# XuyangBai/D3Feat.pytorch

Hardware: AMD Instinct MI355X
Metric: fragment-pairs/sec (fwd+bwd) on 3DMatch-shaped pairs (higher is better)
Workload: dtype f32

## Files before the change

### d3feat.pytorch_amd/_native.py

```python
import ctypes as C
import os
import subprocess

_PKG_DIR = os.path.dirname(os.path.abspath(__file__))
_REPO = os.path.dirname(_PKG_DIR)
LIB_PATH = os.path.join(_PKG_DIR, "libd3feat_hip.so")
CSRC = os.path.join(_PKG_DIR, "csrc")
SOURCES = ["radius_neighbors.hip", "grid_subsample.hip", "kpconv.hip", "kpconv_fused.hip", "kpconv_aggregate.hip", "kpconv_small.hip", "kpconv_deform.hip", "pool.hip", "detection.hip", "loss.hip",
           "reverse_table.hip", "kpconv_dx_gather.hip", "matching.hip", "elementwise.hip", "batchnorm.hip", "linear.hip", "gemm_epilogue.hip", "optimizer.hip", "misc.hip",
           "registration.hip"]

_vp, _i, _f, _sz = C.c_void_p, C.c_int, C.c_float, C.c_size_t


class Tunables(C.Structure):
    _fields_ = [("atb_task_us", C.c_int32), ("atb_form", C.c_int32), ("atb_first_form_wgs", C.c_int32),
                ("match_wgs", C.c_int32), ("agg_through_lds", C.c_int32), ("atb_pipe", C.c_int32), ("xw_rows", C.c_int32), ("xw_split", C.c_int32),
                ("rowgemm_wide", C.c_int32), ("rowgemm_rt", C.c_int32), ("reserved", C.c_int32 * 6)]


class AtbProblem(C.Structure):
    _fields_ = [("x", _vp), ("grad_out", _vp), ("grad_w", _vp), ("N", C.c_int32), ("Cin", C.c_int32),
                ("Cout", C.c_int32), ("ldw", C.c_int32), ("bias_part", _vp), ("bias_blocks", C.c_int32),
                ("bias_cols", C.c_int32), ("grad_bias", _vp), ("grad_bias2", _vp)]


SIGNATURES = {
    "d3f_version": (C.c_char_p, []),
    "d3f_device_arch_ok": (_i, []),
    "d3f_device_arch_name": (_i, [C.c_char_p, _i]),
    "d3f_debug_set_flags": (None, [_i]),
    "d3f_get_tunables": (None, [C.POINTER(Tunables)]),
    "d3f_set_tunables": (_i, [C.POINTER(Tunables)]),
    "d3f_linear_grad_weight_group_ws_bytes": (_sz, [C.POINTER(AtbProblem), _i]),
    "d3f_linear_grad_weight_group": (_i, [C.POINTER(AtbProblem), _i, _vp, _sz, _vp]),
    "d3f_debug_set_phase_clock": (None, [_vp]),
    "d3f_debug_kernel_timing_begin": (_i, [_i, _i]),
    "d3f_debug_kernel_timing_end": (_i, [_vp, _vp, _i]),
    "d3f_radius_grid_ws_bytes": (_sz, [_i]),
    "d3f_radius_grid_build": (_i, [_vp, _i, _vp, _i, _f, _vp, _sz, _vp, _vp]),
    "d3f_radius_query": (_i, [_vp, _vp, _i, _vp, _vp, _i, _vp, _i, _f, _i, _vp, _vp, _vp, _vp, _vp]),
# ... 31 lines not shown
    "d3f_kpconv_aggregate_modes": (_i, [_vp, _i, _vp, _i, _vp, _i, _vp, _i, _vp, _i, _f, _i, _vp, _vp, _vp]),
    "d3f_kpconv_grad_input_modes": (_i, [_vp, _i, _vp, _i, _vp, _i, _i, _vp, _i, _f, _i, _vp, _vp, _vp]),
    "d3f_kpconv_grad_input": (_i, [_vp, _i, _vp, _i, _vp, _i, _vp, _i, _vp, _i, _f, _vp, _vp, _i, _vp, _vp, _sz, _vp]),
    "d3f_kpconv_aggregate_transposed_supported": (_i, [_i, _i]),
    "d3f_kpconv_aggregate_transposed": (_i, [_vp, _i, _i, _i, _vp, _i, _f, _vp, _vp, _i, _vp, _vp]),
    "d3f_reverse_table_ws_bytes": (_sz, [_i, _i, _i]),
    "d3f_reverse_table_build": (_i, [_vp, _i, _i, _i, _vp, _vp, _vp, _sz, _vp]),
    "d3f_kpconv_grad_input_gather_supported": (_i, [_i, _i, _i]),
    "d3f_kpconv_grad_input_gather": (_i, [_vp, _i, _vp, _i, _vp, _vp, _vp, _i, _f, _vp, _vp, _i, _vp, _i, _i, _f, _vp, _vp, _vp,
                                          _vp, _vp]),
    "d3f_reverse_table_filter": (_i, [_vp, _i, _vp, _vp, _i, _vp, _i, _f, _vp, _vp, _vp]),
    "d3f_linear_grad_weight_supported": (_i, [_i, _i, _i]),
    "d3f_linear_fused_supported": (_i, [_i, _i, _i]),
    "d3f_linear_bias_act_forward": (_i, [_vp, _vp, _i, _i, _i, _vp, _vp, _vp, _f, _vp, _vp, _i, _vp]),
    "d3f_linear_pair_supported": (_i, [_i, _i, _i, _i]),
    "d3f_linear_pair_bias_act_forward": (_i, [_vp, _vp, _i, _vp, _vp, _i, _i, _i, _vp, _vp, _vp, _vp, _f, _vp, _vp, _i, _vp]),
    "d3f_linear_grad_input": (_i, [_vp, _vp, _i, _i, _i, _vp, _vp, _vp]),
    "d3f_linear_grad_weight_ws_bytes": (_sz, [_i, _i, _i]),
    "d3f_linear_grad_weight": (_i, [_vp, _vp, _i, _i, _i, _vp, _vp, _sz, _vp]),
    "d3f_linear_grad_weight_bias": (_i, [_vp, _vp, _i, _i, _i, _vp, _vp, _sz, _vp, _i, _i, _vp, _vp, _vp]),
    "d3f_permute_kpconv_weights": (_i, [_vp, _vp, _vp, _vp, _vp, _i, _vp]),
    "d3f_gemm_epilogue_supported": (_i, [_i, _i, _i, _i, _i]),
    "d3f_gemm_epilogue_ws_bytes": (_sz, [_i, _i, _i]),
    "d3f_gemm_epilogue": (_i, [_vp, _i, _vp, _i, _i, _i, _i, _i, _i, _vp, _vp, _vp, _i, _vp, _f, _vp, _i, _vp, _i, _vp, _sz,
                               _vp]),
    "d3f_bias_act_backward_blocks": (_i, [_i, _i]),
    "d3f_bias_act_backward_partial": (_i, [_vp, _vp, _f, _i, _i, _vp, _vp, _vp, _sz, _vp]),
    "d3f_bias_sum": (_i, [_vp, _i, _i, _vp, _vp, _vp]),
    "d3f_max_pool_forward": (_i, [_vp, _i, _i, _vp, _i, _i, _vp, _vp, _vp, _vp, _vp, _i, _i, _vp]),
    "d3f_max_pool_backward": (_i, [_vp, _vp, _i, _i, _i, _vp, _i, _vp]),
    "d3f_closest_pool_forward": (_i, [_vp, _i, _i, _vp, _i, _i, _vp, _i, _vp, _vp, _vp]),
    "d3f_closest_pool_backward": (_i, [_vp, _i, _vp, _i, _i, _i, _i, _vp, _i, _vp]),
    "d3f_bias_act_forward": (_i, [_vp, _vp, _vp, _vp, _f, _i, _i, _vp, _vp, _i, _vp, _vp, _i, _i, _vp]),
    "d3f_bias_act_backward_ws_bytes": (_sz, [_i, _i]),
    "d3f_bias_act_backward": (_i, [_vp, _vp, _f, _i, _i, _vp, _vp, _vp, _i, _vp, _vp, _sz, _vp]),
    "d3f_global_max": (_i, [_vp, _sz, _vp, _vp, _sz, _vp]),
    "d3f_global_max_rows": (_i, [_vp, _i, _i, _vp, _i, _vp, _vp, _sz, _vp]),
    "d3f_global_max_groups": (_i, [_vp, _i, _i, _vp, _i, _i, _vp, _vp, _sz, _vp]),
    "d3f_detection_scores_aux_floats": (_i, [_i]),
    "d3f_detection_scores_forward": (_i, [_vp, _i, _i, _vp, _i, _vp, _i, _vp, _vp, _vp, _vp, _i, _i, _vp]),
    "d3f_detection_scores_ws_bytes": (_sz, [_i, _i]),
    "d3f_detection_scores_backward": (_i, [_vp, _i, _i, _vp, _i, _vp, _vp, _vp, _vp, _vp, _sz, _vp]),
    "d3f_detection_scores_backward_groups": (_i, [_vp, _i, _i, _vp, _i, _vp, _vp, _vp, _vp, _vp, _i, _i, _vp, _sz, _vp]),
    "d3f_circle_det_loss_forward_pairs": (_i, [_vp, _vp, _i, _i, _i, _vp, _vp, _vp, _f, _f, _f, _f, _f, _f, _vp, _vp, _vp,
                                               _vp, _vp, _vp, _vp]),
    "d3f_circle_det_loss_backward_pairs": (_i, [_vp, _vp, _i, _i, _i, _vp, _vp, _vp, _f, _f, _f, _f, _f, _f, _vp, _vp,
# ... 98 lines not shown
        _lib = handle
    return _lib


TRACE = False


def check(rc, what):
    if TRACE:
        import sys
        import torch
        sys.stderr.write("[d3f] %s\n" % what)
        sys.stderr.flush()
        torch.cuda.synchronize()
    if rc != 0:
        raise RuntimeError("%s failed: %s" % (what, ERRORS.get(rc, "error %d" % rc)))


def set_tunables(**kw):
    L = lib()
    t = Tunables()
    L.d3f_get_tunables(C.byref(t))
    old = {name: getattr(t, name) for name, _ in Tunables._fields_ if name != "reserved"}
    for k, v in kw.items():
        if k not in old:
            raise RuntimeError("d3f_tunables has no field %r" % k)
        setattr(t, k, int(v))
    check(L.d3f_set_tunables(C.byref(t)), "d3f_set_tunables")
    return old


def status_message(word):
    return "; ".join(msg for bit, msg in STATUS_BITS.items() if word & bit)
```

### d3feat.pytorch_amd/csrc/gemm_epilogue.hip

```cpp
#include <math.h>

#include "kpconv_tile.hpp"

namespace d3f {

namespace {

constexpr int XW_RING_BYTES = 16 * 1024;
constexpr int XW_LDS_BYTES = 4 * XW_RING_BYTES;

struct XwArgs {
  const float* X;
  const float* W;
  float* Y;
  float* part;
  const float* row_div;
  const float* b1;
  const float* add;
  const float* b2;
  float* zinit;
  int R, Kd, N;
  int lda, ldb, ldy, ldadd;
  int kblock;
  int P, kpp;
// ... 224 lines not shown
  for (int q = 0; q < TI; ++q) {
    const int s = wave * TI + q, i = s >> 2, r = s & 3;
    const int row = m0 + 16 * i + 4 * lk + r;
    float v[TJ];
#pragma unroll
    for (int u = 0; u < TJ; ++u) {
      const int e = ((i * TJ + u) * 4 + r) * 64 + lane;
      v[u] = ((red[e] + red[NT * 256 + e]) + red[2 * NT * 256 + e]) + red[3 * NT * 256 + e];
    }
    if (row < g.R) {
      const int col = n0 + TJ * li;
      if (g.P == 1) {
        xw_epilogue_store<TJ>(v, g, row, col);
      } else {
        float* dst = g.part + ((size_t)p * g.R + row) * g.N + col;
        if constexpr (TJ == 4) *(float4*)dst = make_float4(v[0], v[TJ > 1 ? 1 : 0], v[TJ > 2 ? 2 : 0], v[TJ > 3 ? 3 : 0]);
        else if constexpr (TJ == 2) *(float2*)dst = make_float2(v[0], v[TJ > 1 ? 1 : 0]);
        else dst[0] = v[0];
      }
    }
  }
}

__global__ __launch_bounds__(256) void xw_reduce_epilogue_kernel(const XwArgs g) {
  const size_t e4 = (size_t)blockIdx.x * 256 + threadIdx.x;
  const size_t total4 = (size_t)g.R * g.N / 4;
  if (e4 >= total4) return;
  const float4* part4 = (const float4*)g.part;
  float4 s = part4[e4];
  for (int p = 1; p < g.P; ++p) {
    const float4 w = part4[(size_t)p * total4 + e4];
    s.x += w.x; s.y += w.y; s.z += w.z; s.w += w.w;
  }
  const uint32_t e = (uint32_t)e4 * 4u, row = e / (uint32_t)g.N, col = e - row * (uint32_t)g.N;
  float v[4] = {s.x, s.y, s.z, s.w};
  xw_epilogue_store<4>(v, g, (int)row, (int)col);
}

static inline int xw_tile_width(int n) { return n % 64 == 0 ? 4 : (n % 32 == 0 ? 2 : (n % 16 == 0 ? 1 : 0)); }

struct XwPlan {
  int ti, tj, nrb, nbj, P, kpp;
  unsigned grid;
  size_t slab_floats;
};

}

bool xw_supported(int R, int Kd, int N, int mode, int kblock) {
  if (R < 1 || Kd < 16 || Kd % 16 || N < 16 || !xw_tile_width(N) || mode < 0 || mode > 1) return false;
  if (kblock != 0 && (mode != 0 || kblock < 64 || kblock % 64 || Kd % kblock)) return false;
  if (((size_t)R + 64) * (size_t)Kd * 4 >= 0xfff00000ull || ((size_t)N + 64) * (size_t)Kd * 4 >= 0xfff00000ull) return false;
  if ((size_t)R * N >= 0x3fffffffull) return false;
  return true;
}

static XwPlan xw_plan(int R, int Kd, int N) {
  XwPlan a;
  const d3f_tunables& tn = tunables();
  a.tj = xw_tile_width(N);
  a.nbj = N / (16 * a.tj);
  a.ti = 4;
  if ((long long)cdiv(R, 64) * a.nbj < 512) a.ti = 2;
  if (tn.xw_rows == 2 || tn.xw_rows == 4) a.ti = tn.xw_rows;
  a.nrb = cdiv(R, 16 * a.ti);
  const long long ntiles = (long long)a.nrb * a.nbj;
  a.P = 1;
  if (ntiles <= 160 && Kd >= 1024 && Kd % 128 == 0) a.P = 8;
  if (tn.xw_split == 1) a.P = 1;
  if (tn.xw_split >= 8 && tn.xw_split % 8 == 0 && Kd % (16 * tn.xw_split) == 0) a.P = tn.xw_split;
  a.kpp = a.P == 1 ? Kd : Kd / a.P;
  a.grid = a.P == 1 ? (unsigned)(8 * ((ntiles + 7) / 8)) : (unsigned)(a.P * ntiles);
  a.slab_floats = a.P == 1 ? 0 : (size_t)a.P * R * N;
  return a;
}

size_t xw_ws_bytes(int R, int Kd, int N) {
  return 256 + align_up(sizeof(float) * xw_plan(R, Kd, N).slab_floats, 256);
}

int xw_gemm(const float* X, int lda, const float* W, int ldb, int mode, int kblock, int R, int Kd, int N,
            const float* row_div, const float* b1, const float* add, int ldadd, const float* b2, float slope, float* Y,
            int ldy, float* zinit, int zn, void* ws, size_t ws_bytes, hipStream_t stream) {
  if (!X || !W || !Y || !xw_supported(R, Kd, N, mode, kblock)) return D3F_EINVAL;
  if (lda < Kd || ldy < N || (add && ldadd < N) || (zinit && zn < 1)) return D3F_EINVAL;
  if (mode == 0 && kblock == 0 && ldb < Kd) return D3F_EINVAL;
  if (mode == 1 && ldb < N) return D3F_EINVAL;
  if ((((uintptr_t)X | (uintptr_t)W | (uintptr_t)Y | (uintptr_t)add | (uintptr_t)b1 | (uintptr_t)b2) & 15) != 0) return D3F_EINVAL;
  if ((lda | ldb | ldy | (add ? ldadd : 0)) & 3) return D3F_EINVAL;
  const XwPlan pl = xw_plan(R, Kd, N);
  if (pl.P > 1 && (!ws || ws_bytes < xw_ws_bytes(R, Kd, N))) return D3F_EWORKSPACE;
  XwArgs g;
  g.X = X; g.W = W; g.Y = Y;
  g.part = pl.P > 1 ? (float*)ws : nullptr;
  g.row_div = row_div; g.b1 = b1; g.add = add; g.b2 = b2;
  g.zinit = zinit; g.zn = zinit ? zn : 0;
  g.R = R; g.Kd = Kd; g.N = N;
  g.lda = lda; g.ldb = (mode == 0 && kblock > 0) ? kblock : ldb; g.ldy = ldy; g.ldadd = add ? ldadd : 0;
  g.kblock = kblock;
  g.P = pl.P; g.kpp = pl.kpp;
  g.nrb = pl.nrb; g.nbj = pl.nbj;
  g.slope = slope;
  const size_t bx = (size_t)R * lda * 4;
  const size_t bw = mode == 1 ? (size_t)Kd * ldb * 4 : (kblock > 0 ? (size_t)Kd * N * 4 : (size_t)N * ldb * 4);
  if (bx >= 0xfff00000ull || bw >= 0xfff00000ull) return D3F_EINVAL;
  g.bytesX = (unsigned)bx;
  g.bytesW = (unsigned)bw;
#define D3F_XW(I, J, M) \
  case (M) * 64 + (I) * 8 + (J): xw_gemm_kernel<I, J, M><<<pl.grid, 256, XW_LDS_BYTES, stream>>>(g); break
  switch (mode * 64 + pl.ti * 8 + pl.tj) {
    D3F_XW(2, 1, 0); D3F_XW(2, 2, 0); D3F_XW(2, 4, 0); D3F_XW(4, 1, 0); D3F_XW(4, 2, 0); D3F_XW(4, 4, 0);
    D3F_XW(2, 1, 1); D3F_XW(2, 2, 1); D3F_XW(2, 4, 1); D3F_XW(4, 1, 1); D3F_XW(4, 2, 1); D3F_XW(4, 4, 1);
    default: return D3F_EINVAL;
  }
#undef D3F_XW
  D3F_LAUNCH_CHECK();
  if (pl.P > 1) {
    xw_reduce_epilogue_kernel<<<cdiv((long long)R * N / 4, 256), 256, 0, stream>>>(g);
    D3F_LAUNCH_CHECK();
  }
  return D3F_OK;
}

}

extern "C" {

int d3f_gemm_epilogue_supported(int R, int K, int N, int mode, int kblock) {
  return d3f::xw_supported(R, K, N, mode, kblock) ? 1 : 0;
}

size_t d3f_gemm_epilogue_ws_bytes(int R, int K, int N) {
  if (R < 1 || K < 16 || N < 16) return 0;
  return d3f::xw_ws_bytes(R, K, N);
}

int d3f_gemm_epilogue(const float* x, int ldx, const float* w, int ldw, int mode, int kblock, int R, int K, int N,
                      const float* row_div, const float* bias1, const float* add, int ldadd, const float* bias2,
                      float slope, float* y, int ldy, float* zero_init, int zero_n, void* ws, size_t ws_bytes,
                      void* stream) {
  return d3f::xw_gemm(x, ldx, w, ldw, mode, kblock, R, K, N, row_div, bias1, add, ldadd, bias2, slope, y, ldy, zero_init,
                      zero_n, ws, ws_bytes, (hipStream_t)stream);
}

}
```

### d3feat.pytorch_amd/csrc/misc.hip

```cpp
#include <string.h>

#include "common.hpp"

namespace {

struct CopyJobs {
  const void* src[24];
  void* dst[24];
  size_t n[24];
  int kind[24];
  double thr;
};
__global__ __launch_bounds__(256) void copy_many_kernel(CopyJobs jobs) {
  const int j = blockIdx.y;
  const size_t stride = (size_t)gridDim.x * blockDim.x, t0 = (size_t)blockIdx.x * blockDim.x + threadIdx.x;
  const size_t n = jobs.n[j];
  if (jobs.kind[j] == 0) {
    const uint32_t* s = (const uint32_t*)jobs.src[j];
    uint32_t* d = (uint32_t*)jobs.dst[j];
    for (size_t i = t0; i < n; i += stride) d[i] = s[i];
  } else {
    const double* s = (const double*)jobs.src[j];
    uint8_t* d = (uint8_t*)jobs.dst[j];
    for (size_t i = t0; i < n; i += stride) d[i] = s[i] > jobs.thr ? 1 : 0;
// ... 22 lines not shown
    __syncthreads();
#pragma unroll
    for (int i = 0; i < 4; ++i) d[(size_t)(ly + 8 * i) * Cin + lx] = tile[lx][ly + 8 * i];
    __syncthreads();
  }
}

}

namespace d3f {
static d3f_tunables g_tunables = {};
const d3f_tunables& tunables() { return g_tunables; }
}

extern "C" {

void d3f_get_tunables(d3f_tunables* out) {
  if (out) *out = d3f::g_tunables;
}
int d3f_set_tunables(const d3f_tunables* in) {
  if (!in || in->atb_task_us < 0 || in->atb_form < 0 || in->atb_form > 2 || in->atb_first_form_wgs < 0 ||
      in->match_wgs < 0 || in->atb_pipe < 0 || in->atb_pipe > 16 || in->xw_rows < 0 || in->xw_rows > 4 || in->xw_split < 0 ||
      in->xw_split > 64 || in->rowgemm_wide < 0 || in->rowgemm_wide > 2 ||
      in->rowgemm_rt < 0 || in->rowgemm_rt > 1)
    return D3F_EINVAL;
  d3f::g_tunables = *in;
  return D3F_OK;
}

int d3f_copy_buffers(const void* const* srcs, void* const* dsts, const size_t* bytes, const int* kinds, int n,
                     double threshold, void* stream) {
  if (n < 0 || n > 24 || (n > 0 && (!srcs || !dsts || !bytes || !kinds))) return D3F_EINVAL;
  CopyJobs jobs;
  jobs.thr = threshold;
  int m = 0;
  size_t most = 0;
  for (int j = 0; j < n; ++j) {
    if (bytes[j] == 0) continue;
    if (!srcs[j] || !dsts[j] || (kinds[j] != 0 && kinds[j] != 1)) return D3F_EINVAL;
    if (kinds[j] == 0 && (((uintptr_t)srcs[j] | (uintptr_t)dsts[j] | bytes[j]) & 3)) return D3F_EINVAL;
    if (kinds[j] == 1 && (((uintptr_t)srcs[j] | bytes[j]) & 7)) return D3F_EINVAL;
    jobs.src[m] = srcs[j];
    jobs.dst[m] = dsts[j];
    jobs.n[m] = kinds[j] == 0 ? bytes[j] / 4 : bytes[j] / 8;
    jobs.kind[m] = kinds[j];
    if (jobs.n[m] > most) most = jobs.n[m];
    ++m;
// ... 63 lines not shown
```

### d3feat.pytorch_amd/ops.py

```python
import numpy as np
import ctypes
import threading

import torch

from . import _native

ORDER_REFERENCE = 0
ORDER_FIRST_SEEN = 1


def _stream():
    return torch.cuda.current_stream().cuda_stream


_PROFILER = None


def set_profiler(p):
    global _PROFILER
    _PROFILER = p


class _Region:
# ... 918 lines not shown
        return False
    return bool(_native.lib().d3f_gemm_epilogue_supported(int(R), int(K), int(N), int(mode), int(kblock)))


def gemm_epilogue(x, w, mode, R, K, N, kblock=0, ldx=None, ldw=None, row_div=None, bias1=None, add=None, bias2=None,
                  slope=1.0, zero_init=None, out=None):
    L = _native.lib()
    ldx = K if ldx is None else int(ldx)
    ldw = (K if mode == GEMM_NT else N) if ldw is None else int(ldw)
    if out is None:
        out = torch.empty((R, N), dtype=torch.float32, device=x.device)
    ldy = int(out.stride(0)) if out.dim() == 2 else N
    ldadd = int(add.stride(0)) if add is not None else 0
    nbytes = int(L.d3f_gemm_epilogue_ws_bytes(int(R), int(K), int(N)))
    ws = _ws(nbytes, x.device)
    zn = int(zero_init.numel()) if zero_init is not None else 0
    with _region("gemm_epilogue[R=%d,K=%d,N=%d,mode=%d]" % (R, K, N, mode), 4 * (R * K + K * N + R * N)):
        _native.check(L.d3f_gemm_epilogue(_p(x), ldx, _p(w), ldw, int(mode), int(kblock), int(R), int(K), int(N),
                                          _p(row_div), _p(bias1), _p(add), ldadd, _p(bias2), float(slope), _p(out), ldy,
                                          _p(zero_init), zn, _p(ws), nbytes, _stream()), "d3f_gemm_epilogue")
    return out


OWN_GEMM_KINDS = {"kpconv_fwd"}
OWN_GEMM_RULES = True
OWN_GEMM_TALL_ROWS = 1 << 30


def _own_gemm(kind, x, w, mode, R, K, N, kblock=0, ldx=None, ldw=None, *others):
    if kind not in OWN_GEMM_KINDS:
        return False
    if OWN_GEMM_RULES:
        if kind == "kpconv_fwd" and not (R <= 1024 or 4096 <= R < 16384 or R >= OWN_GEMM_TALL_ROWS):
            return False
        if kind in ("unary_fwd", "unary_dx") and R < 16384:
            return False
        if kind == "kpconv_dx" and R > 1024:
            return False
    return gemm_epilogue_ok(x, w, mode, R, K, N, kblock, ldx, ldw, *others)


class _LinearFn(torch.autograd.Function):
    @staticmethod
    def forward(ctx, x, weight, holder=None, deposit=None):
        ctx.save_for_backward(x, weight)
        ctx.gw_slot = _grad_slot(weight)
        ctx.holder, ctx.dep = holder, deposit
        return torch.mm(x, weight.t())

    @staticmethod
    def backward(ctx, grad_out):
        x, weight = ctx.saved_tensors
        go = grad_out.contiguous()
        gx = _add_deposited(ctx.holder, go, weight) if ctx.needs_input_grad[0] else None
        if gx is not None and ctx.dep is not None and ctx.dep.deposit(gx):
            gx = None
        gw = None
        if ctx.needs_input_grad[1]:
# ... 1258 lines not shown
```

### include/d3feat_hip.h

```cpp
#ifndef D3FEAT_HIP_H_
#define D3FEAT_HIP_H_

#include <stddef.h>
#include <stdint.h>

#ifdef __cplusplus
extern "C" {
#endif

#define D3F_OK 0
#define D3F_EINVAL (-1)
#define D3F_EWORKSPACE (-2)
#define D3F_ELAUNCH (-3)

#define D3F_ST_CAND_OVERFLOW 1
#define D3F_ST_CELL_RANGE 2
#define D3F_ST_TABLE_FULL 4
#define D3F_ST_CAPACITY 8
#define D3F_ST_WIDE_OVERFLOW 16
#define D3F_ST_NO_NEAREST 32

const char* d3f_version(void);
int d3f_device_arch_ok(void);
int d3f_device_arch_name(char* out, int n);
void d3f_debug_set_flags(int flags);
void d3f_debug_set_phase_clock(void* counters);
int d3f_debug_kernel_timing_begin(int which, int max_launches);
int d3f_debug_kernel_timing_end(float* ms_out, int32_t* shapes_out, int cap);

typedef struct d3f_tunables {
  int32_t atb_task_us;
  int32_t atb_form;
  int32_t atb_first_form_wgs;
  int32_t match_wgs;
  int32_t agg_through_lds;
  int32_t atb_pipe;
  int32_t xw_rows;
  int32_t xw_split;
  int32_t rowgemm_wide;
  int32_t rowgemm_rt;
  int32_t reserved[6];
} d3f_tunables;
void d3f_get_tunables(d3f_tunables* out);
int d3f_set_tunables(const d3f_tunables* in);

size_t d3f_radius_grid_ws_bytes(int Ns);
int d3f_radius_grid_build(const float* supports, int Ns, const int32_t* s_len, int B, float radius,
                          void* grid_ws, size_t grid_ws_bytes, int32_t* status, void* stream);
size_t d3f_radius_grid_zero_bytes(int Ns);
int d3f_zero_buffers(void* const* ptrs, const size_t* bytes, int n, void* stream);
int d3f_copy_buffers(const void* const* srcs, void* const* dsts, const size_t* bytes, const int* kinds, int n,
                     double threshold, void* stream);
int d3f_radius_query_prefix_missing(const void* grid_ws, const float* queries, int Nq, const int32_t* q_len, int Ns,
                                    const int32_t* s_len, int B, float grid_radius, float radius, float prefix_radius,
                                    float nearest_bound, int width, int32_t* out_idx, const int32_t* done_rows,
                                    int32_t* status, void* stream);
int d3f_radius_query_pool_transposed(const void* grid_ws, const float* queries, int Nq, const int32_t* q_len, int Ns,
                                     const int32_t* s_len, int B, float grid_radius, float radius, int width,
                                     int32_t* out_idx, int32_t* max_count, uint64_t* out_last_key, int max_count_group,
                                     int32_t* tr_counts, uint64_t* tr_keys, int32_t* status, void* stream);
int d3f_upsample_rows_rank(int32_t* counts, const uint64_t* keys, int Nf, int Nc, int width, int32_t* up,
                           void* stream);
int d3f_radius_grid_build_prezeroed(const float* supports, int Ns, const int32_t* s_len, int B, float radius,
                                    void* grid_ws, size_t grid_ws_bytes, int32_t* status, void* stream);
// ... 57 lines not shown
                          const void* spack_kept, int grad_x_precleared, float* grad_x, void* ws, size_t ws_bytes,
                          void* stream);
int d3f_kpconv_aggregate_transposed_supported(int Cout, int K);
int d3f_kpconv_aggregate_transposed(const float* rev_rel, int rev_width, int Ns, int Nq, const float* kernel_points,
                                    int K, float extent, const float* nn, const float* grad_out, int Cout,
                                    float* agg_out, void* stream);

int d3f_linear_grad_weight_supported(int N, int Cin, int Cout);
int d3f_linear_fused_supported(int N, int Cin, int Cout);
int d3f_linear_bias_act_forward(const float* x, const float* weight, int N, int Cin, int Cout, const float* bias1,
                                const float* add, const float* bias2, float slope, float* out, float* zero_init,
                                int zero_n, void* stream);
int d3f_linear_pair_supported(int N, int Cin1, int Cin2, int Cout);
int d3f_linear_pair_bias_act_forward(const float* x1, const float* w1, int Cin1, const float* x2, const float* w2, int Cin2,
                                     int N, int Cout, const float* bias1, const float* bias2, const float* bias3,
                                     const float* bias4, float slope, float* out, float* zero_init, int zero_n,
                                     void* stream);
int d3f_linear_grad_input(const float* grad_out, const float* weight, int N, int Cin, int Cout, const float* add,
                          float* grad_x, void* stream);
int d3f_permute_kpconv_weights(const float* const* srcs_host, float* const* dsts_host, const int* K_host,
                               const int* Cin_host, const int* Cout_host, int n, void* stream);
int d3f_gemm_epilogue_supported(int R, int K, int N, int mode, int kblock);
size_t d3f_gemm_epilogue_ws_bytes(int R, int K, int N);
int d3f_gemm_epilogue(const float* x, int ldx, const float* w, int ldw, int mode, int kblock, int R, int K, int N,
                      const float* row_div, const float* bias1, const float* add, int ldadd, const float* bias2,
                      float slope, float* y, int ldy, float* zero_init, int zero_n, void* ws, size_t ws_bytes,
                      void* stream);
size_t d3f_linear_grad_weight_ws_bytes(int N, int Cin, int Cout);
int d3f_linear_grad_weight(const float* x, const float* grad_out, int N, int Cin, int Cout, float* grad_w, void* ws,
                           size_t ws_bytes, void* stream);
int d3f_linear_grad_weight_bias(const float* x, const float* grad_out, int N, int Cin, int Cout, float* grad_w, void* ws,
                                size_t ws_bytes, const float* bias_part, int bias_blocks, int bias_cols,
                                float* grad_bias, float* grad_bias2, void* stream);
typedef struct d3f_atb_problem {
  const float* x;
  const float* grad_out;
  float* grad_w;
  int32_t N, Cin, Cout, ldw;
  const float* bias_part;
  int32_t bias_blocks, bias_cols;
  float* grad_bias;
  float* grad_bias2;
} d3f_atb_problem;
size_t d3f_linear_grad_weight_group_ws_bytes(const d3f_atb_problem* problems_host, int n);
int d3f_linear_grad_weight_group(const d3f_atb_problem* problems_host, int n, void* ws, size_t ws_bytes, void* stream);

// ... 148 lines not shown
```

### profiles/gemm_epilogue_bench.py

```python
import argparse
import os
import sys

import numpy as np
import torch

sys.path.insert(0, os.path.dirname(os.path.dirname(os.path.abspath(__file__))))
from d3feat_pytorch_amd import _native, ops

NT, NN = ops.GEMM_NT, ops.GEMM_NN
SHAPES = [
    ("kpconv fwd L1", 23808, 960, 64, NN, 0, 'fk'), ("kpconv fwd L2s", 6208, 960, 64, NN, 0, 'fk'),
    ("kpconv fwd L2", 6208, 1920, 128, NN, 0, 'fk'), ("kpconv fwd L3s", 1792, 1920, 128, NN, 0, 'fk'),
    ("kpconv fwd L3", 1792, 3840, 256, NN, 0, 'fk'), ("kpconv fwd L4s", 512, 3840, 256, NN, 0, 'fk'),
    ("kpconv fwd L4", 512, 7680, 512, NN, 0, 'fk'),
    ("unary L0 128>32", 114624, 128, 32, NT, 0, 'f'), ("unary L1 128>64", 23808, 128, 64, NT, 0, 'f'),
    ("unary L1 128>256", 23808, 128, 256, NT, 0, 'f'), ("unary L1 256>64", 23808, 256, 64, NT, 0, 'f'),
    ("unary L2 256>128", 6208, 256, 128, NT, 0, 'f'), ("unary L2 256>512", 6208, 256, 512, NT, 0, 'f'),
    ("unary L2 128>512", 6208, 128, 512, NT, 0, 'f'), ("unary L2 512>128", 6208, 512, 128, NT, 0, 'f'),
    ("unary L3 128>512", 1792, 128, 512, NT, 0, 'f'), ("unary L3 512>256", 1792, 512, 256, NT, 0, 'f'),
    ("unary L3 512>1024", 1792, 512, 1024, NT, 0, 'f'), ("unary L3 256>1024", 1792, 256, 1024, NT, 0, 'f'),
    ("unary L3 1024>256", 1792, 1024, 256, NT, 0, 'f'), ("unary L4 256>1024", 512, 256, 1024, NT, 0, 'f'),
    ("unary L4 1024>512", 512, 1024, 512, NT, 0, 'f'), ("unary L4 1024>2048", 512, 1024, 2048, NT, 0, 'f'),
    ("unary L4 512>2048", 512, 512, 2048, NT, 0, 'f'), ("unary L4 2048>512", 512, 2048, 512, NT, 0, 'f'),
# ... 29 lines not shown
    torch.cuda.synchronize()
    e0, e1 = torch.cuda.Event(enable_timing=True), torch.cuda.Event(enable_timing=True)
    e0.record()
    for _ in range(3):
        g.replay()
    e1.record()
    torch.cuda.synchronize()
    return e0.elapsed_time(e1) * 1e3 / (3 * reps)


def main():
    ap = argparse.ArgumentParser()
    ap.add_argument("--reps", type=int, default=30)
    ap.add_argument("--variants", action="store_true")
    ap.add_argument("--out", default=None)
    ap.add_argument("--no-table", action="store_true", help="library GEMMs on their default picks (no TunableOp table)")
    args = ap.parse_args()
    if not args.no_table:
        import d3feat_pytorch_amd
        print("# TunableOp table loaded:", d3feat_pytorch_amd.enable_tuned_gemms())
    L = _native.lib()
    rng = np.random.default_rng(3)
    lines = []
    variants = [(0, 0)] + ([(2, 1), (4, 1), (2, 8), (4, 8), (2, 16), (4, 16)] if args.variants else [])
    head = "%-20s %7s %5s %5s %2s | %8s %8s | " % ("shape", "R", "K", "N", "m", "lib", "lib+epi") + " ".join(
        "%9s" % ("own" if v == (0, 0) else "r%d/s%d" % v) for v in variants) + " |  TF(own)  best"
    print(head)
    lines.append(head)
    tot_lib = tot_libepi = tot_own = 0.0
    for label, R, K, N, mode, kblock, epi in SHAPES:
        x = torch.from_numpy(rng.normal(size=(R, K)).astype(np.float32)).cuda()
        if kblock:
            Kp = K // kblock
            W3 = torch.from_numpy(rng.normal(size=(Kp, N, kblock)).astype(np.float32)).cuda()
            w = W3
            b_lib = W3.permute(0, 2, 1).reshape(K, N).contiguous()
            lib_mm = lambda: torch.mm(x, W3.permute(0, 2, 1).contiguous().view(K, N))
        elif mode == NT:
            w = torch.from_numpy(rng.normal(size=(N, K)).astype(np.float32)).cuda()
            b_lib = w.t()
            lib_mm = lambda: torch.mm(x, w.t())
        else:
            w = torch.from_numpy(rng.normal(size=(K, N)).astype(np.float32)).cuda()
            b_lib = w
            lib_mm = lambda: torch.mm(x, w)
        row_div = torch.from_numpy(rng.integers(1, 40, size=R).astype(np.float32)).cuda() if 'k' in epi else None
        bias = torch.from_numpy(rng.normal(size=N).astype(np.float32)).cuda() if 'f' in epi else None
        addend = torch.from_numpy(rng.normal(size=(R, N)).astype(np.float32)).cuda() if 'a' in epi else None
        slope = 0.1 if 'f' in epi else 1.0
        out = torch.empty((R, N), device="cuda")
        def lib_epi():
            if addend is not None:
                return torch.addmm(addend, x, b_lib)
            raw = lib_mm()
            if 'f' in epi:
                _native.check(L.d3f_bias_act_forward(raw.data_ptr(), bias.data_ptr(), None, None, slope, R, N, out.data_ptr(), None,
                                                     0, row_div.data_ptr() if row_div is not None else None, None, 0, 0,
                                                     torch.cuda.current_stream().cuda_stream), "ba")
            return raw

        def own():
            ops.gemm_epilogue(x, w, mode, R, K, N, kblock, None, None, row_div, bias, addend, None, slope, None, out)

        t_lib = timed(lib_mm, args.reps)
        t_libepi = timed(lib_epi, args.reps)
        ts = []
        for v in variants:
            old = _native.set_tunables(xw_rows=v[0], xw_split=v[1])
            try:
                ts.append(timed(own, args.reps))
            finally:
                _native.set_tunables(**old)
        ref = x.double() @ b_lib.double()
        if row_div is not None:
            ref = ref / row_div.double()[:, None]
        if bias is not None:
            ref = ref + bias.double()
        if addend is not None:
            ref = ref + addend.double()
        ref = torch.where(ref > 0, ref, ref * slope)
        own()
        err = float((out.double() - ref).abs().max() / ref.abs().max())
        flop = 2.0 * R * K * N
        best = int(np.argmin(ts))
        line = "%-20s %7d %5d %5d %2d | %8.1f %8.1f | " % (label, R, K, N, mode, t_lib, t_libepi) + " ".join(
            "%9.1f" % t for t in ts) + " | %6.1f  %s  err %.1e" % (flop / ts[0] * 1e-6, "own" if best == 0 else "r%d/s%d" % variants[best], err)
        print(line, flush=True)
        lines.append(line)
        tot_lib += t_lib
        tot_libepi += t_libepi
        tot_own += ts[0]
    tail = "# totals (each shape once): library %.1f us, library + epilogue %.1f us, own %.1f us" % (tot_lib, tot_libepi, tot_own)
    print(tail)
    lines.append(tail)
    if args.out:
        with open(args.out, "w") as f:
            f.write("\n".join(lines) + "\n")


if __name__ == "__main__":
    main()
```

Measured before the change: 686.0.

## Add shared-tile 3-slot pipelined MFMA GEMM and route more GEMMs to it

```diff
diff --git a/d3feat.pytorch_amd/_native.py b/d3feat.pytorch_amd/_native.py
--- a/d3feat.pytorch_amd/_native.py
+++ b/d3feat.pytorch_amd/_native.py
@@ -17,6 +17,9 @@
     _fields_ = [("atb_task_us", C.c_int32), ("atb_form", C.c_int32), ("atb_first_form_wgs", C.c_int32),
                 ("match_wgs", C.c_int32), ("agg_through_lds", C.c_int32), ("atb_pipe", C.c_int32), ("xw_rows", C.c_int32), ("xw_split", C.c_int32),
                 ("rowgemm_wide", C.c_int32), ("rowgemm_rt", C.c_int32), ("reserved", C.c_int32 * 6)]
+
+
+_RESERVED_NAMES = {"xw_tile": 0}
 
 
 class AtbProblem(C.Structure):
@@ -94,6 +97,7 @@
     "d3f_permute_kpconv_weights": (_i, [_vp, _vp, _vp, _vp, _vp, _i, _vp]),
     "d3f_gemm_epilogue_supported": (_i, [_i, _i, _i, _i, _i]),
     "d3f_gemm_epilogue_ws_bytes": (_sz, [_i, _i, _i]),
+    "d3f_gemm_epilogue_plan": (_i, [_i, _i, _i, _vp]),
     "d3f_gemm_epilogue": (_i, [_vp, _i, _vp, _i, _i, _i, _i, _i, _i, _vp, _vp, _vp, _i, _vp, _f, _vp, _i, _vp, _i, _vp, _sz,
                                _vp]),
     "d3f_bias_act_backward_blocks": (_i, [_i, _i]),
@@ -238,10 +242,15 @@
     t = Tunables()
     L.d3f_get_tunables(C.byref(t))
     old = {name: getattr(t, name) for name, _ in Tunables._fields_ if name != "reserved"}
+    for name, slot in _RESERVED_NAMES.items():
+        old[name] = t.reserved[slot]
     for k, v in kw.items():
         if k not in old:
             raise RuntimeError("d3f_tunables has no field %r" % k)
-        setattr(t, k, int(v))
+        if k in _RESERVED_NAMES:
+            t.reserved[_RESERVED_NAMES[k]] = int(v)
+        else:
+            setattr(t, k, int(v))
     check(L.d3f_set_tunables(C.byref(t)), "d3f_set_tunables")
     return old
 
diff --git a/d3feat.pytorch_amd/csrc/gemm_epilogue.hip b/d3feat.pytorch_amd/csrc/gemm_epilogue.hip
--- a/d3feat.pytorch_amd/csrc/gemm_epilogue.hip
+++ b/d3feat.pytorch_amd/csrc/gemm_epilogue.hip
@@ -270,6 +270,198 @@
   }
 }
 
+constexpr int XS_SLOTS = 3;
+
+template <int TI, int TJ, int MODE>
+__global__ __launch_bounds__(256, 2) void xw_gemm_shared_kernel(const XwArgs g) {
+  constexpr int BM = 32 * TI, BN = 32 * TJ;
+  constexpr int A_BYTES = 2 * TI * 1024, SB = A_BYTES + 2 * TJ * 1024;
+  constexpr int GA = TI / 2, GB = TJ / 2, GW = GA + GB;
+  constexpr int NRB = (MODE == 1) ? 4 : TJ;
+  constexpr int NRD = TI + NRB;
+  constexpr int NM = 4 * TI * TJ, EXTRAS = GW + NRD;
+  static_assert(TI % 2 == 0 && TJ % 2 == 0, "every wave issues the same number of pieces");
+  const int lane = threadIdx.x & 63, wave = __builtin_amdgcn_readfirstlane((int)(threadIdx.x >> 6));
+  const int wr = wave >> 1, wc = wave & 1;
+  const int li = lane & 15, lk = lane >> 4;
+  if (g.zinit && blockIdx.x == 0)
+    for (int t = threadIdx.x; t < g.zn; t += 256) g.zinit[t] = 0.0f;
+  const int L = blockIdx.x;
+  const int ntiles = g.nrb * g.nbj;
+  int p = 0, tile;
+  if (g.P == 1) {
+    const int per = (ntiles + 7) >> 3;
+    tile = (L & 7) * per + (L >> 3);
+    if ((L >> 3) >= per || tile >= ntiles) return;
+  } else {
+    p = (L & 7) + 8 * ((L >> 3) / ntiles);
+    tile = (L >> 3) % ntiles;
+    if (p >= g.P) return;
+  }
+  const int rb = tile / g.nbj, cb = tile - rb * g.nbj;
+  const int m0 = rb * BM, n0 = cb * BN;
+  const int k0 = p * g.kpp, k1 = min(g.Kd, k0 + g.kpp);
+  const int ngroups = (k1 - k0) >> 4;
+  const unsigned ring_addr = __builtin_amdgcn_readfirstlane((unsigned)(uintptr_t)xw_smem);
+  const __amdgpu_buffer_rsrc_t rsA = __builtin_amdgcn_make_buffer_rsrc(const_cast<float*>(g.X), 0, g.bytesX, 0x00020000);
+  const __amdgpu_buffer_rsrc_t rsB = __builtin_amdgcn_make_buffer_rsrc(const_cast<float*>(g.W), 0, g.bytesW, 0x00020000);
+  unsigned voA[GA], voB[GB];
+#pragma unroll
+  for (int s = 0; s < GA; ++s)
+    voA[s] = (unsigned)(((size_t)min(m0 + 16 * (4 * s + wave) + li, g.R - 1) * g.lda + 4 * lk) * 4);
+#pragma unroll
+  for (int s = 0; s < GB; ++s) {
+    const int xb = 4 * s + wave, c = xb / TJ, j = xb % TJ, nq = n0 + 16 * TJ * c;
+    if constexpr (MODE == 0) {
+      voB[s] = (unsigned)(((size_t)(nq + TJ * li + j) * g.ldb + 4 * lk) * 4);
+    } else {
+      const int e = j * 64 + lane, row = e / (4 * TJ), col = (e % (4 * TJ)) * 4;
+      voB[s] = (unsigned)(((size_t)row * g.ldb + nq + col) * 4);
+    }
+  }
+  const int kblk = (MODE == 0 && g.kblock > 0) ? g.kblock : 0x40000000;
+  const unsigned blk_bytes = (MODE == 0 && g.kblock > 0) ? (unsigned)g.N * (unsigned)g.kblock * 4u : 0u;
+  int kq = k0;
+  int kb = kq / kblk;
+  int ko = kq - kb * kblk;
+  unsigned sA = 0, sB = 0;
+  auto group_offsets = [&]() {
+    sA = (unsigned)kq * 4u;
+    if constexpr (MODE == 0) sB = (unsigned)kb * blk_bytes + (unsigned)ko * 4u;
+    else sB = (unsigned)kq * (unsigned)g.ldb * 4u;
+  };
+  auto next_group = [&]() {
+    kq += 16;
+    ko += 16;
+    const bool wrap = ko >= kblk;
+    ko = wrap ? ko - kblk : ko;
+    kb = wrap ? kb + 1 : kb;
+    group_offsets();
+  };
+  group_offsets();
+
+  f32x4 acc[TI][TJ];
+#pragma unroll
+  for (int i = 0; i < TI; ++i)
+#pragma unroll
+    for (int u = 0; u < TJ; ++u) acc[i][u] = (f32x4){0.f, 0.f, 0.f, 0.f};
+
+  auto dma_piece = [&](int x, int slot) {
+    const unsigned sa = ring_addr + (unsigned)slot * SB;
+#pragma unroll
+    for (int s = 0; s < GA; ++s)
+      if (x == s)
+        xw_dma16(rsA, voA[s], __builtin_amdgcn_readfirstlane(sA),
+                 __builtin_amdgcn_readfirstlane(sa + (4 * s + wave) * 1024));
+#pragma unroll
+    for (int s = 0; s < GB; ++s)
+      if (x == GA + s)
+        xw_dma16(rsB, voB[s], __builtin_amdgcn_readfirstlane(sB),
+                 __builtin_amdgcn_readfirstlane(sa + A_BYTES + (4 * s + wave) * 1024));
+    if (x == GW - 1) next_group();
+  };
+  auto read_frag = [&](int y, int slot, float (&a)[TI][4], float (&b)[4][TJ]) {
+    const unsigned char* s0 = xw_smem + slot * SB;
+    const unsigned char* sa = s0 + wr * (TI * 1024);
+    const unsigned char* sb = s0 + A_BYTES + wc * (TJ * 1024);
+#pragma unroll
+    for (int i = 0; i < TI; ++i)
+      if (y == i) {
+        const float4 v = *(const float4*)(sa + i * 1024 + lane * 16);
+        a[i][0] = v.x; a[i][1] = v.y; a[i][2] = v.z; a[i][3] = v.w;
+      }
+    if constexpr (MODE == 0) {
+#pragma unroll
+      for (int u = 0; u < TJ; ++u)
+        if (y == TI + u) {
+          const float4 v = *(const float4*)(sb + u * 1024 + lane * 16);
+          b[0][u] = v.x; b[1][u] = v.y; b[2][u] = v.z; b[3][u] = v.w;
+        }
+    } else {
+      const float* sBf = (const float*)sb;
+#pragma unroll
+      for (int ks = 0; ks < 4; ++ks)
+        if (y == TI + ks) {
+          const typename VecT<TJ>::type v = *(const typename VecT<TJ>::type*)(sBf + (4 * lk + ks) * (16 * TJ) + TJ * li);
+#pragma unroll
+          for (int u = 0; u < TJ; ++u) b[ks][u] = vget<TJ>(v, u);
+        }
+    }
+  };
+  auto block = [&](float (&a)[TI][4], float (&b)[4][TJ], float (&a2)[TI][4], float (&b2)[4][TJ], int slot, int nslot,
+                   bool do_dma) {
+#pragma unroll
+    for (int m = 0; m < NM; ++m) {
+      const int ks = m / (TI * TJ), u = (m / TI) % TJ, i = m % TI;
+      acc[i][u] = __builtin_amdgcn_mfma_f32_16x16x4f32(a[i][ks], b[ks][u], acc[i][u], 0, 0, 0);
+#pragma unroll
+      for (int e = 0; e < (EXTRAS + NM - 1) / NM; ++e) {
+        const int x = (m * EXTRAS) / NM + e;
+        if (x >= ((m + 1) * EXTRAS) / NM) continue;
+        if (x < GW) {
+          if (do_dma) dma_piece(x, slot);
+        } else {
+          read_frag(x - GW, nslot, a2, b2);
+        }
+        __builtin_amdgcn_sched_barrier(0);
+      }
+    }
+  };
+  auto sync_slot = [&](int it) {
+    if (it + 2 < ngroups) asm volatile("s_waitcnt vmcnt(%0) lgkmcnt(0)\n\ts_barrier" ::"n"(GW) : "memory");
+    else asm volatile("s_waitcnt vmcnt(0) lgkmcnt(0)\n\ts_barrier" ::: "memory");
+  };
+
+  if (ngroups > 0) {
+    float a0[TI][4], b0[4][TJ], a1[TI][4], b1[4][TJ];
+#pragma unroll
+    for (int x = 0; x < GW; ++x) dma_piece(x, 0);
+    if (ngroups > 1) {
+#pragma unroll
+      for (int x = 0; x < GW; ++x) dma_piece(x, 1);
+    }
+    if (ngroups > 2) {
+#pragma unroll
+      for (int x = 0; x < GW; ++x) dma_piece(x, 2);
+    }
+    sync_slot(-1);
+#pragma unroll
+    for (int y = 0; y < NRD; ++y) read_frag(y, 0, a0, b0);
+    __builtin_amdgcn_sched_barrier(0);
+    int slot = 0;
+    for (int it = 0; it < ngroups; it += 2) {
+      sync_slot(it);
+      const int s1 = slot == XS_SLOTS - 1 ? 0 : slot + 1;
+      block(a0, b0, a1, b1, slot, s1, it + 3 < ngroups);
+      if (it + 1 < ngroups) {
+        sync_slot(it + 1);
+        const int s2 = s1 == XS_SLOTS - 1 ? 0 : s1 + 1;
+        block(a1, b1, a0, b0, s1, s2, it + 4 < ngroups);
+        slot = s2;
+      }
+    }
+  }
+
+#pragma unroll
+  for (int i = 0; i < TI; ++i)
+#pragma unroll
+    for (int r = 0; r < 4; ++r) {
+      const int row = m0 + 16 * TI * wr + 16 * i + 4 * lk + r;
+      if (row >= g.R) continue;
+      const int col = n0 + 16 * TJ * wc + TJ * li;
+      float v[TJ];
+#pragma unroll
+      for (int u = 0; u < TJ; ++u) v[u] = acc[i][u][r];
+      if (g.P == 1) {
+        xw_epilogue_store<TJ>(v, g, row, col);
+      } else {
+        float* dst = g.part + ((size_t)p * g.R + row) * g.N + col;
+        if constexpr (TJ == 4) *(float4*)dst = make_float4(v[0], v[TJ > 1 ? 1 : 0], v[TJ > 2 ? 2 : 0], v[TJ > 3 ? 3 : 0]);
+        else *(float2*)dst = make_float2(v[0], v[TJ > 1 ? 1 : 0]);
+      }
+    }
+}
+
 __global__ __launch_bounds__(256) void xw_reduce_epilogue_kernel(const XwArgs g) {
   const size_t e4 = (size_t)blockIdx.x * 256 + threadIdx.x;
   const size_t total4 = (size_t)g.R * g.N / 4;
@@ -288,8 +480,9 @@
 static inline int xw_tile_width(int n) { return n % 64 == 0 ? 4 : (n % 32 == 0 ? 2 : (n % 16 == 0 ? 1 : 0)); }
 
 struct XwPlan {
+  int shared;
   int ti, tj, nrb, nbj, P, kpp;
-  unsigned grid;
+  unsigned grid, lds;
   size_t slab_floats;
 };
 
@@ -306,19 +499,39 @@
 static XwPlan xw_plan(int R, int Kd, int N) {
   XwPlan a;
   const d3f_tunables& tn = tunables();
+  const int form = tn.xw_tile;
+  auto split_of = [&](long long ntiles) {
+    int P = 1;
+    if (ntiles <= 160 && Kd >= 1024 && Kd % 128 == 0) P = 8;
+    if (tn.xw_split == 1) P = 1;
+    if (tn.xw_split >= 8 && tn.xw_split % 8 == 0 && Kd % (16 * tn.xw_split) == 0) P = tn.xw_split;
+    return P;
+  };
+  a.shared = 0;
   a.tj = xw_tile_width(N);
-  a.nbj = N / (16 * a.tj);
-  a.ti = 4;
-  if ((long long)cdiv(R, 64) * a.nbj < 512) a.ti = 2;
+  a.ti = (long long)cdiv(R, 64) * (N / (16 * a.tj)) < 512 ? 2 : 4;
   if (tn.xw_rows == 2 || tn.xw_rows == 4) a.ti = tn.xw_rows;
-  a.nrb = cdiv(R, 16 * a.ti);
+  a.P = split_of((long long)cdiv(R, 16 * a.ti) * (N / (16 * a.tj)));
+  if (form != 1 && N % 64 == 0) {
+    const long long t64 = (long long)cdiv(R, 64) * (N / 64);
+    bool take = form >= 2;
+    if (form == 0)
+      take = t64 >= 256 || (a.P == 8 && split_of(t64) == 8 && Kd < 3072 && tn.xw_split == 0);
+    const int tj = form == 4 ? 4 : 2;
+    if (take && N % (32 * tj) == 0) {
+      a.shared = 1;
+      a.ti = (tn.xw_rows == 2 || tn.xw_rows == 4) ? tn.xw_rows : 2;
+      a.tj = tj;
+      a.P = split_of((long long)cdiv(R, 32 * a.ti) * (N / (32 * a.tj)));
+    }
+  }
+  const int bm = (a.shared ? 32 : 16) * a.ti, bn = (a.shared ? 32 : 16) * a.tj;
+  a.nrb = cdiv(R, bm);
+  a.nbj = N / bn;
   const long long ntiles = (long long)a.nrb * a.nbj;
-  a.P = 1;
-  if (ntiles <= 160 && Kd >= 1024 && Kd % 128 == 0) a.P = 8;
-  if (tn.xw_split == 1) a.P = 1;
-  if (tn.xw_split >= 8 && tn.xw_split % 8 == 0 && Kd % (16 * tn.xw_split) == 0) a.P = tn.xw_split;
   a.kpp = a.P == 1 ? Kd : Kd / a.P;
   a.grid = a.P == 1 ? (unsigned)(8 * ((ntiles + 7) / 8)) : (unsigned)(a.P * ntiles);
+  a.lds = a.shared ? (unsigned)(XS_SLOTS * (2 * a.ti + 2 * a.tj) * 1024) : (unsigned)XW_LDS_BYTES;
   a.slab_floats = a.P == 1 ? 0 : (size_t)a.P * R * N;
   return a;
 }
@@ -355,12 +568,23 @@
   g.bytesX = (unsigned)bx;
   g.bytesW = (unsigned)bw;
 #define D3F_XW(I, J, M) \
-  case (M) * 64 + (I) * 8 + (J): xw_gemm_kernel<I, J, M><<<pl.grid, 256, XW_LDS_BYTES, stream>>>(g); break
-  switch (mode * 64 + pl.ti * 8 + pl.tj) {
-    D3F_XW(2, 1, 0); D3F_XW(2, 2, 0); D3F_XW(2, 4, 0); D3F_XW(4, 1, 0); D3F_XW(4, 2, 0); D3F_XW(4, 4, 0);
-    D3F_XW(2, 1, 1); D3F_XW(2, 2, 1); D3F_XW(2, 4, 1); D3F_XW(4, 1, 1); D3F_XW(4, 2, 1); D3F_XW(4, 4, 1);
-    default: return D3F_EINVAL;
-  }
+  case (M) * 64 + (I) * 8 + (J): xw_gemm_kernel<I, J, M><<<pl.grid, 256, pl.lds, stream>>>(g); break
+#define D3F_XS(I, J, M) \
+  case (M) * 64 + (I) * 8 + (J): xw_gemm_shared_kernel<I, J, M><<<pl.grid, 256, pl.lds, stream>>>(g); break
+  if (pl.shared) {
+    switch (mode * 64 + pl.ti * 8 + pl.tj) {
+      D3F_XS(2, 2, 0); D3F_XS(2, 4, 0); D3F_XS(4, 2, 0); D3F_XS(4, 4, 0);
+      D3F_XS(2, 2, 1); D3F_XS(2, 4, 1); D3F_XS(4, 2, 1); D3F_XS(4, 4, 1);
+      default: return D3F_EINVAL;
+    }
+  } else {
+    switch (mode * 64 + pl.ti * 8 + pl.tj) {
+      D3F_XW(2, 1, 0); D3F_XW(2, 2, 0); D3F_XW(2, 4, 0); D3F_XW(4, 1, 0); D3F_XW(4, 2, 0); D3F_XW(4, 4, 0);
+      D3F_XW(2, 1, 1); D3F_XW(2, 2, 1); D3F_XW(2, 4, 1); D3F_XW(4, 1, 1); D3F_XW(4, 2, 1); D3F_XW(4, 4, 1);
+      default: return D3F_EINVAL;
+    }
+  }
+#undef D3F_XS
 #undef D3F_XW
   D3F_LAUNCH_CHECK();
   if (pl.P > 1) {
@@ -381,6 +605,13 @@
 size_t d3f_gemm_epilogue_ws_bytes(int R, int K, int N) {
   if (R < 1 || K < 16 || N < 16) return 0;
   return d3f::xw_ws_bytes(R, K, N);
+}
+
+int d3f_gemm_epilogue_plan(int R, int K, int N, int* plan) {
+  if (!plan || !d3f::xw_supported(R, K, N, 0, 0)) return D3F_EINVAL;
+  const d3f::XwPlan pl = d3f::xw_plan(R, K, N);
+  plan[0] = pl.shared; plan[1] = pl.ti; plan[2] = pl.tj; plan[3] = pl.P; plan[4] = (int)pl.lds; plan[5] = (int)pl.grid;
+  return D3F_OK;
 }
 
 int d3f_gemm_epilogue(const float* x, int ldx, const float* w, int ldw, int mode, int kblock, int R, int K, int N,
diff --git a/d3feat.pytorch_amd/csrc/misc.hip b/d3feat.pytorch_amd/csrc/misc.hip
--- a/d3feat.pytorch_amd/csrc/misc.hip
+++ b/d3feat.pytorch_amd/csrc/misc.hip
@@ -68,7 +68,7 @@
   if (!in || in->atb_task_us < 0 || in->atb_form < 0 || in->atb_form > 2 || in->atb_first_form_wgs < 0 ||
       in->match_wgs < 0 || in->atb_pipe < 0 || in->atb_pipe > 16 || in->xw_rows < 0 || in->xw_rows > 4 || in->xw_split < 0 ||
       in->xw_split > 64 || in->rowgemm_wide < 0 || in->rowgemm_wide > 2 ||
-      in->rowgemm_rt < 0 || in->rowgemm_rt > 1)
+      in->rowgemm_rt < 0 || in->rowgemm_rt > 1 || in->xw_tile < 0 || in->xw_tile > 4)
     return D3F_EINVAL;
   d3f::g_tunables = *in;
   return D3F_OK;
diff --git a/d3feat.pytorch_amd/ops.py b/d3feat.pytorch_amd/ops.py
--- a/d3feat.pytorch_amd/ops.py
+++ b/d3feat.pytorch_amd/ops.py
@@ -964,9 +964,13 @@
     return out
 
 
-OWN_GEMM_KINDS = {"kpconv_fwd"}
+OWN_GEMM_KINDS = {"kpconv_fwd", "unary_fwd", "unary_dx", "decoder"}
 OWN_GEMM_RULES = True
 OWN_GEMM_TALL_ROWS = 1 << 30
+
+
+def _blocks64(R, N):
+    return -(-R // 64) * (N // 64) if N % 64 == 0 else 0
 
 
 def _own_gemm(kind, x, w, mode, R, K, N, kblock=0, ldx=None, ldw=None, *others):
@@ -975,7 +979,11 @@
     if OWN_GEMM_RULES:
         if kind == "kpconv_fwd" and not (R <= 1024 or 4096 <= R < 16384 or R >= OWN_GEMM_TALL_ROWS):
             return False
-        if kind in ("unary_fwd", "unary_dx") and R < 16384:
+        if kind == "unary_fwd" and not (R >= 16384 or (_blocks64(R, N) >= 384 and K <= 512) or (K <= 256 and N >= 512)):
+            return False
+        if kind == "unary_dx" and not (R >= 1024 and K >= 256 and N <= 512):
+            return False
+        if kind == "decoder" and not (mode == GEMM_NT and _blocks64(R, N) >= 700 and K >= 256):
             return False
         if kind == "kpconv_dx" and R > 1024:
             return False
diff --git a/include/d3feat_hip.h b/include/d3feat_hip.h
--- a/include/d3feat_hip.h
+++ b/include/d3feat_hip.h
@@ -39,7 +39,8 @@
   int32_t xw_split;
   int32_t rowgemm_wide;
   int32_t rowgemm_rt;
-  int32_t reserved[6];
+  int32_t xw_tile;
+  int32_t reserved[5];
 } d3f_tunables;
 void d3f_get_tunables(d3f_tunables* out);
 int d3f_set_tunables(const d3f_tunables* in);
@@ -143,6 +144,7 @@
                                const int* Cin_host, const int* Cout_host, int n, void* stream);
 int d3f_gemm_epilogue_supported(int R, int K, int N, int mode, int kblock);
 size_t d3f_gemm_epilogue_ws_bytes(int R, int K, int N);
+int d3f_gemm_epilogue_plan(int R, int K, int N, int* plan);
 int d3f_gemm_epilogue(const float* x, int ldx, const float* w, int ldw, int mode, int kblock, int R, int K, int N,
                       const float* row_div, const float* bias1, const float* add, int ldadd, const float* bias2,
                       float slope, float* y, int ldy, float* zero_init, int zero_n, void* ws, size_t ws_bytes,
diff --git a/profiles/gemm_epilogue_bench.py b/profiles/gemm_epilogue_bench.py
--- a/profiles/gemm_epilogue_bench.py
+++ b/profiles/gemm_epilogue_bench.py
@@ -1,4 +1,5 @@
 import argparse
+import ctypes
 import os
 import sys
 
@@ -75,12 +76,26 @@
     L = _native.lib()
     rng = np.random.default_rng(3)
     lines = []
-    variants = [(0, 0)] + ([(2, 1), (4, 1), (2, 8), (4, 8), (2, 16), (4, 16)] if args.variants else [])
+    variants = [("own", {}, None)]
+    if args.variants:
+        variants.append(("private", dict(xw_tile=1), None))
+        for ti, tj in ((4, 4), (4, 2), (2, 4), (2, 2)):
+            for split in (1, 8):
+                variants.append(("%dx%d/s%d" % (32 * ti, 32 * tj, split),
+                                 dict(xw_tile=4 if tj == 4 else 3, xw_rows=ti, xw_split=split), (ti, tj)))
+    plan = (ctypes.c_int * 6)()
+
+    def plan_of(R, K, N):
+        _native.check(L.d3f_gemm_epilogue_plan(R, K, N, plan), "plan")
+        return list(plan)
+
     head = "%-20s %7s %5s %5s %2s | %8s %8s | " % ("shape", "R", "K", "N", "m", "lib", "lib+epi") + " ".join(
-        "%9s" % ("own" if v == (0, 0) else "r%d/s%d" % v) for v in variants) + " |  TF(own)  best"
+        "%9s" % v[0] for v in variants) + " |  TF(own)  best       plan"
     print(head)
     lines.append(head)
     tot_lib = tot_libepi = tot_own = 0.0
+    n_win = 0
+    tot_var = None
     for label, R, K, N, mode, kblock, epi in SHAPES:
         x = torch.from_numpy(rng.normal(size=(R, K)).astype(np.float32)).cuda()
         if kblock:
@@ -118,12 +133,19 @@
         t_lib = timed(lib_mm, args.reps)
         t_libepi = timed(lib_epi, args.reps)
         ts = []
-        for v in variants:
-            old = _native.set_tunables(xw_rows=v[0], xw_split=v[1])
+        for _, tun, want in variants:
+            old = _native.set_tunables(**tun)
             try:
-                ts.append(timed(own, args.reps))
+                pl = plan_of(R, K, N)
+                if want is not None and (pl[0] != 1 or (pl[1], pl[2]) != want):
+                    ts.append(float("nan"))
+                else:
+                    ts.append(timed(own, args.reps))
             finally:
                 _native.set_tunables(**old)
+        pl = plan_of(R, K, N)
+        bm, bn = (32 if pl[0] else 16) * pl[1], (32 if pl[0] else 16) * pl[2]
+        plan_s = "%s%dx%d/s%d" % ("s" if pl[0] else "p", bm, bn, pl[3])
         ref = x.double() @ b_lib.double()
         if row_div is not None:
             ref = ref / row_div.double()[:, None]
@@ -135,15 +157,23 @@
         own()
         err = float((out.double() - ref).abs().max() / ref.abs().max())
         flop = 2.0 * R * K * N
-        best = int(np.argmin(ts))
+        best = int(np.nanargmin(ts))
         line = "%-20s %7d %5d %5d %2d | %8.1f %8.1f | " % (label, R, K, N, mode, t_lib, t_libepi) + " ".join(
-            "%9.1f" % t for t in ts) + " | %6.1f  %s  err %.1e" % (flop / ts[0] * 1e-6, "own" if best == 0 else "r%d/s%d" % variants[best], err)
+            "%9s" % ("-" if t != t else "%.1f" % t) for t in ts) + " | %6.1f  %-9s %-12s err %.1e" % (
+            flop / ts[0] * 1e-6, variants[best][0], plan_s, err)
         print(line, flush=True)
         lines.append(line)
         tot_lib += t_lib
         tot_libepi += t_libepi
         tot_own += ts[0]
-    tail = "# totals (each shape once): library %.1f us, library + epilogue %.1f us, own %.1f us" % (tot_lib, tot_libepi, tot_own)
+        n_win += int(ts[0] <= t_libepi)
+        if args.variants:
+            tot_var = [a + b for a, b in zip(tot_var, ts)] if tot_var else list(ts)
+    tail = "# totals (each shape once): library %.1f us, library + epilogue %.1f us, own %.1f us; own <= library + epilogue " \
+           "on %d of %d shapes" % (tot_lib, tot_libepi, tot_own, n_win, len(SHAPES))
+    if args.variants:
+        tail += "\n# variant totals ('-' shapes count as nan): " + ", ".join(
+            "%s %.1f" % (v[0], t) for v, t in zip(variants, tot_var))
     print(tail)
     lines.append(tail)
     if args.out:
```

After: 685.6 (median of 3 runs). About the same (-0.1%).
